# fpusan/moira

Measured on AMD Instinct MI355X. Metric: reads/sec filtered (300 bp synthetic), higher is better.
Workload: dtype f64; 1 GPU; BASELINE configs[1]: 10000000 synthetic single-end 300 bp reads, poisson_binomial filter, alpha 0.005, uncert 0.01, resident in HBM (uint8 10000000 x 320, seed 2); reads_per_gpu=10000000, read_length=300, row_stride=320, parallelism=host-side split, 1 rank(s), no data-path collective, world_size=1, mode=bit-exact (no FMA)

## Files before the change

### include/moira_pb.h

```cpp
#ifndef MOIRA_PB_H
#define MOIRA_PB_H

#include <stdint.h>

#ifdef __cplusplus
extern "C" {
#endif
#if defined(__GNUC__) || defined(__clang__)
#pragma GCC visibility push(default)
#endif

#define MPB_OK            0
#define MPB_E_INVALID    -1
#define MPB_E_NODEVICE   -2
#define MPB_E_HIP        -3
#define MPB_E_NOMEM      -4
#define MPB_E_RANGE      -5

#define MPB_AMBIG_TREAT_AS_ERRORS 0
#define MPB_AMBIG_IGNORE          1
#define MPB_AMBIG_DISALLOW        2

#define MPB_FLAG_ROUND      1u
#define MPB_FLAG_FAST_FMA   2u
// ... 167 lines not shown
int mpb_broker_attach(const char *name, int32_t wait_ms, mpb_broker_client **client_out);
int mpb_broker_call(mpb_broker_client *client, const char *contig, const int32_t *contig_quals, int32_t len,
                    double alpha, double *ee, int32_t *ns);
int mpb_broker_detach(mpb_broker_client *client);
int mpb_broker_shutdown(const char *name);
int mpb_broker_stats(const char *name, int64_t *served, int64_t *batches, int64_t *solo, int32_t *pid, int32_t *attached);

int mpb_numa_cpulist_for_pci(const char *sysfs_root, const char *pci_bus_id, int32_t *node_out, char *cpulist_out, int32_t cpulist_len);

int mpb_poisson_lambda_device(mpb_ctx *ctx, const uint8_t *d_q, int64_t n, int64_t row_stride,
                              const int32_t *d_len, int32_t fixed_len,
                              double *d_lambda, int32_t *d_ns);
int mpb_poisson_finish_host(const double *lambda, const int32_t *ns, const int32_t *len,
                            int32_t fixed_len, int64_t n, const mpb_filter_params *params,
                            double *ee, uint8_t *pass);
int mpb_filter_poisson_host(mpb_ctx *ctx, const uint8_t *q, int64_t n, int64_t row_stride,
                            const int32_t *len, int32_t fixed_len, const mpb_filter_params *params,
                            double *ee, int32_t *ns, uint8_t *pass, mpb_filter_counts *counts);

int mpb_poisson_finish_device(mpb_ctx *ctx, const double *d_lambda, const int32_t *d_ns,
                              const int32_t *d_len, int32_t fixed_len, int64_t n,
                              const mpb_filter_params *params,
                              double *d_ee, uint8_t *d_pass, mpb_filter_counts *counts);
int mpb_filter_poisson_device(mpb_ctx *ctx, const uint8_t *d_q, int64_t n, int64_t row_stride,
                              const int32_t *d_len, int32_t fixed_len,
                              const mpb_filter_params *params,
                              double *d_ee, int32_t *d_ns, uint8_t *d_pass, double *d_lambda,
                              mpb_filter_counts *counts);

int mpb_calculate_errors_poisson(mpb_ctx *ctx, const char *sequence,
                                 const int32_t *quals, int32_t len,
                                 double alpha, double *ee, int32_t *ns);

int mpb_synth_fill_device(mpb_ctx *ctx, uint8_t *d_q, int64_t n, int64_t row_stride,
                          int32_t fixed_len, int32_t min_len, int32_t max_len,
                          int32_t *d_len, uint64_t seed, int64_t first_read);
int mpb_synth_fill_device_profile(mpb_ctx *ctx, uint8_t *d_q, int64_t n, int64_t row_stride,
                                  int32_t fixed_len, int32_t min_len, int32_t max_len,
                                  int32_t *d_len, uint64_t seed, int64_t first_read, int32_t profile);

int mpb_timing_enable(mpb_ctx *ctx, int on);
int mpb_timing_reset(mpb_ctx *ctx);
int mpb_kernel_time(mpb_ctx *ctx, int kernel_id, double *total_ms, int64_t *launches);
int mpb_last_class_histogram(mpb_ctx *ctx, int32_t *caps, int64_t *counts, int32_t max_classes);
int mpb_last_read_budgets(mpb_ctx *ctx, int32_t *caps_out, int64_t n);
int mpb_last_algorithmic_cells(mpb_ctx *ctx, int64_t *cells);

typedef struct mpb_path_info {
    int32_t narrow_rows;
    int32_t sampled;
    int64_t n_fallback;
    int32_t sample_hist[16];
    int32_t narrow_split;
    int32_t reserved_;
} mpb_path_info;
int mpb_last_path(mpb_ctx *ctx, mpb_path_info *out);

#if defined(__GNUC__) || defined(__clang__)
#pragma GCC visibility pop
#endif
#ifdef __cplusplus
}
#endif
#endif
```

### moira_amd/_lib.py

```python
import ctypes as C
import os

_HERE = os.path.dirname(os.path.abspath(__file__))
LIB_PATH = os.path.join(_HERE, "libmoira_pb.so")

MAX_LEN = 65535
OK, E_INVALID, E_NODEVICE, E_HIP, E_NOMEM, E_RANGE = 0, -1, -2, -3, -4, -5
AMBIG = {"treat_as_errors": 0, "ignore": 1, "disallow": 2}
FLAG_ROUND, FLAG_FAST_FMA, FLAG_TEST_UNDERPREDICT, FLAG_DECISION_ONLY, FLAG_BATCHED_ONLY, FLAG_COUNT_CELLS = 1, 2, 4, 8, 16, 32
FLAG_NO_NARROW = 64
FLAG_ODDS = 128
FLAG_ODDS_NARROW = 1 << 20
FLAG_POISSON_DEVICE_TAIL = 1 << 21


def FLAG_NARROW_ROWS(r):
    return (int(r) & 15) << 8


K_PREPASS, K_SCAN, K_SCATTER, K_DP, K_OVERFLOW, K_LAMBDA, K_WIDE, K_NARROW, K_FALLBACK, K_SAMPLE = 0, 1, 2, 3, 4, 5, 6, 7, 8, 9
K_POISSON_TAIL = 10
K_PACK_TEXT = 11
KERNEL_NAMES = {K_PREPASS: "prepass", K_SCAN: "scan", K_SCATTER: "scatter", K_DP: "dp", K_OVERFLOW: "overflow", K_LAMBDA: "lambda",
                K_WIDE: "wide", K_NARROW: "narrow", K_FALLBACK: "fallback", K_SAMPLE: "sample", K_POISSON_TAIL: "poisson_tail",
                K_PACK_TEXT: "pack_text"}


class MoiraPBError(RuntimeError):
    pass


class NoDeviceError(MoiraPBError):
    pass


class FilterParams(C.Structure):
    _fields_ = [("alpha", C.c_double), ("uncert", C.c_double), ("maxerrors", C.c_double),
                ("ambig_mode", C.c_int32), ("flags", C.c_uint32)]


class PathInfo(C.Structure):
    _fields_ = [("narrow_rows", C.c_int32), ("sampled", C.c_int32), ("n_fallback", C.c_int64),
                ("sample_hist", C.c_int32 * 16), ("narrow_split", C.c_int32), ("reserved_", C.c_int32)]


class FilterCounts(C.Structure):
    _fields_ = [("n_reads", C.c_int64), ("n_pass", C.c_int64), ("n_fail", C.c_int64),
                ("n_overflow", C.c_int64)]


class TextRow(C.Structure):
    _fields_ = [("seq_off", C.c_int64), ("qual_off", C.c_int64), ("len", C.c_int32), ("pad", C.c_int32)]


class PairRow(C.Structure):
    _fields_ = [("fseq_off", C.c_int64), ("fqual_off", C.c_int64), ("fhdr_off", C.c_int64), ("rseq_off", C.c_int64),
                ("rqual_off", C.c_int64), ("l1", C.c_int32), ("l2", C.c_int32), ("hdr_len", C.c_int32), ("pad", C.c_int32)]


class ContigParams(C.Structure):
    _fields_ = [(k, C.c_int32) for k in ("match", "mismatch", "gap", "insert", "deltaq", "consensus", "qscore_cap", "trim_overlap")]


CONTIG_MAX_LEN = 384

_VP, _I32P, _U8P, _DP = C.c_void_p, C.POINTER(C.c_int32), C.POINTER(C.c_uint8), C.POINTER(C.c_double)
PROTOTYPES = {
    "mpb_version": (C.c_char_p, []),
    "mpb_last_error": (C.c_char_p, []),
    "mpb_device_count": (C.c_int, []),
    "mpb_create": (C.c_int, [C.c_int, C.POINTER(_VP)]),
    "mpb_destroy": (C.c_int, [_VP]),
    "mpb_host_lut": (C.c_int, [_VP, _VP]),
    "mpb_device_lut": (C.c_int, [_VP, _VP, _VP]),
    "mpb_stream": (C.c_int, [_VP, C.POINTER(_VP)]),
    "mpb_synchronize": (C.c_int, [_VP]),
    "mpb_malloc": (C.c_int, [_VP, C.c_int64, C.POINTER(_VP)]),
    "mpb_free": (C.c_int, [_VP, _VP]),
    "mpb_memcpy_h2d": (C.c_int, [_VP, _VP, _VP, C.c_int64]),
    "mpb_memcpy_d2h": (C.c_int, [_VP, _VP, _VP, C.c_int64]),
    "mpb_memset": (C.c_int, [_VP, _VP, C.c_int, C.c_int64]),
    "mpb_host_alloc": (C.c_int, [_VP, C.c_int64, C.POINTER(_VP)]),
    "mpb_host_free": (C.c_int, [_VP, _VP]),
    "mpb_pack_read": (C.c_int, [C.c_char_p, _VP, C.c_int32, _VP, C.c_int32]),
    "mpb_pack_read_ascii": (C.c_int, [C.c_char_p, C.c_char_p, C.c_int32, C.c_int32, _VP, C.c_int32]),
    "mpb_pack_batch_ascii": (C.c_int, [C.c_char_p, C.c_char_p, _VP, C.c_int64, C.c_int32, C.c_int32, C.c_int64, _VP, _VP]),
    "mpb_decode_ascii_device": (C.c_int, [_VP, _VP, _VP, C.c_int64, C.c_int64, _VP, C.c_int32, C.c_int32, _VP, _VP]),
    "mpb_text_rows": (C.c_int, [_VP, C.c_int64, _VP, C.c_int64, C.c_int64, C.c_int32, C.c_int64, _VP, C.POINTER(C.c_int64),
                                C.POINTER(C.c_int64)]),
    "mpb_pack_text_device": (C.c_int, [_VP, _VP, C.c_int64, _VP, C.c_int64, C.c_int32, C.c_int32, C.c_int64, _VP, _VP, _VP, _VP]),
    "mpb_filter_text_host": (C.c_int, [_VP, _VP, C.c_int64, _VP, C.c_int64, _VP, C.c_int64, C.c_int32, C.c_int32, C.c_int32,
                                       C.POINTER(FilterParams), C.c_int32, _VP, _VP, _VP, _VP, _VP, C.POINTER(FilterCounts),
                                       C.POINTER(C.c_int64)]),
    "mpb_pair_rows": (C.c_int, [_VP, _VP, C.c_int64, C.c_int64, C.c_int64, C.c_int64, _VP, C.POINTER(C.c_int64)]),
    "mpb_contig_posterior_tables": (C.c_int, [_VP, _VP]),
    "mpb_contigs_text_host": (C.c_int, [_VP, _VP, C.c_int64, _VP, _VP, C.c_int64, _VP, C.c_int64, C.c_int32, C.POINTER(ContigParams),
# ... 95 lines not shown
```

### moira_amd/build.py

```python
import fcntl
import hashlib
import os
import subprocess
import sys

HERE = os.path.dirname(os.path.abspath(__file__))
ROOT = os.path.dirname(HERE)
CSRC = os.path.join(HERE, "csrc")
LIB = os.path.join(HERE, "libmoira_pb.so")
HOST_SOURCES = [os.path.join(CSRC, name) for name in ("mpb_hostonly.cpp", "mpb_context.cpp", "mpb_resident.cpp", "mpb_hostfed.cpp",
                                                      "mpb_perread.cpp", "mpb_poisson.cpp", "mpb_text.cpp", "mpb_contig.cpp",
                                                      "mpb_broker.cpp")]
CONTIG_KERNELS = os.path.join(CSRC, "mpb_contig_kernels.hip")
SOURCES = [os.path.join(CSRC, "mpb_kernels.hip"), CONTIG_KERNELS] + HOST_SOURCES
DEPS = SOURCES + [os.path.join(CSRC, "mpb_internal.h"), os.path.join(CSRC, "mpb_host_internal.h"),
                  os.path.join(CSRC, "mpb_shared.h"), os.path.join(CSRC, "mpb_hostonly.h"), os.path.join(CSRC, "mpb_ctx.h"),
                  os.path.join(CSRC, "mpb_dp_tiles.inc"),
                  os.path.join(CSRC, "mpb_narrow_ring.inc"), os.path.join(CSRC, "mpb_narrow_rs.inc"),
                  os.path.join(CSRC, "mpb_narrow_rg.inc"),
                  os.path.join(CSRC, "mpb_contig_lane.inc"), os.path.join(CSRC, "mpb_contig_args.h"),
                  os.path.join(CSRC, "contig_posterior.h"),
                  os.path.join(CSRC, "libmoira_pb.map"),
                  os.path.join(ROOT, "include", "moira_pb.h"),
                  os.path.join(ROOT, "include", "mpb_synth.h")]
HIPCC = os.environ.get("HIPCC", "/opt/rocm/bin/hipcc")
FLAGS = ["-O3", "--offload-arch=gfx950", "-fPIC", "-shared", "-std=c++17",
         "-ffp-contract=off", "-fno-fast-math", "-pthread", "-Wall", "-Wno-unused-function",
         "-Werror=pass-failed",
         "-fvisibility=hidden",
         "-Wl,--version-script=" + os.path.join(CSRC, "libmoira_pb.map"),
         "-x", "hip"]


CONTIG_LIB = os.path.join(HERE, "libmoira_contig.so")
CONTIG_SRC = os.path.join(CSRC, "contig.cpp")
CXX = os.environ.get("CXX", "g++")


CONTIG_DEPS = [CONTIG_SRC, os.path.join(CSRC, "contig_posterior.h"), os.path.join(ROOT, "include", "moira_contig.h"),
               os.path.join(ROOT, "include", "moira_io.h")]


def _digest(paths, flags):
    h = hashlib.sha256(" ".join(flags).encode())
    for p in paths:
        with open(p, "rb") as f:
            h.update(f.read())
    return h.hexdigest()


def _is_stale(lib, deps, flags):
    stamp = lib + ".stamp"
    if not os.path.exists(lib) or not os.path.exists(stamp):
        return True
    try:
        return open(stamp).read().strip() != _digest(deps, flags)
    except OSError:
        return True


def _locked_build(lib, deps, flags, cmd, force, verbose):
    with open(lib + ".lock", "w") as lk:
        fcntl.flock(lk, fcntl.LOCK_EX)
        try:
            if force or _is_stale(lib, deps, flags):
                if verbose:
                    print(" ".join(cmd))
                tmp = lib + ".tmp.%d" % os.getpid()
                subprocess.check_call(cmd[:-1] + [tmp])
                os.replace(tmp, lib)
                with open(lib + ".stamp", "w") as f:
                    f.write(_digest(deps, flags))
                if verbose:
# ... 71 lines not shown
```

### moira_amd/csrc/mpb_internal.h

```cpp
#ifndef MPB_INTERNAL_H
#define MPB_INTERNAL_H

#include <hip/hip_runtime.h>
#include "mpb_shared.h"

#define MPB_TILE_MAX_ROWS 1024
#define MPB_WIDE_WAVES 16
#define MPB_MAX_ROWS (MPB_TILE_MAX_ROWS * MPB_WIDE_WAVES)
#define MPB_MAX_STRIDE 65536
#define MPB_SMALL_MAX_STRIDE 16384

struct MpbClass { int cap, G, R; };

#define MPB_NCLS 32
#define MPB_CLASSES(X)                                                                       \
    X(0, 2, 1) X(1, 3, 1) X(2, 4, 1) X(3, 5, 1) X(4, 6, 1) X(5, 7, 1) X(6, 8, 1) X(7, 9, 1)  \
    X(8, 10, 1) X(9, 12, 1) X(10, 14, 1) X(11, 16, 1)                                        \
    X(12, 10, 2) X(13, 12, 2) X(14, 14, 2) X(15, 16, 2)                                      \
    X(16, 10, 4) X(17, 12, 4) X(18, 14, 4) X(19, 16, 4)                                      \
    X(20, 9, 8) X(21, 10, 8) X(22, 11, 8) X(23, 12, 8) X(24, 14, 8) X(25, 16, 8)             \
    X(26, 10, 16) X(27, 12, 16) X(28, 16, 16)                                                \
    X(29, 12, 32) X(30, 16, 32) X(31, 16, 64)

#define MPB_THIN_CLASSES(X)                                                                  \
// ... 22 lines not shown
};

#define MPB_DP_CHUNK 8

struct MpbDevParams {
    double thr;
    double uncert;
    double maxerrors;
    float  z;
    float  zq;
    float  clow;
    int32_t ambig_mode;
    uint32_t flags;
    int32_t fixed_len;
    int32_t max_len;
    int32_t len_shift;
};

struct MpbWorkspace {
    uint8_t  *cls;
    int32_t  *perm;
    uint16_t *perm_ns;
    int32_t  *blockhist;
    MpbTables *tables;
    MpbTables *tables2;
    int32_t  *ovf_list;
    int32_t  *ovf_count;
    int32_t  *bad_len;
    long long *ovf_total;
    int32_t  *wide_list;
    int32_t  *wide_rows;
    int32_t  *wide_count;
    unsigned long long *pass_count;
    unsigned long long *alg_cells;
    const double2 *lut;
    int32_t  *nar_count;
    int32_t  *nar_seg;
    int32_t  *nar_list;
    int32_t  *nar_wave_count;
    int32_t  *nar_sample;
    int2     *rg_ord;
    int32_t  *rg_gpre;
    unsigned long long *rg_wsum, *rg_wpre;
    int32_t  *rg_gstart;
    int32_t  *pt_count;
};

#define MPB_NAR_MAX_WAVES 8192
#define MPB_NAR_AUTO_MIN_READS (1 << 18)

#define MPB_LUT_BYTES   (256 * 16)
#define MPB_LAMBDA_MAX_STRIDE (1 << 24)

void mpb_launch_prepass(const uint8_t *q, int64_t n, int64_t stride, const int32_t *len,
                        const MpbDevParams &prm, const MpbWorkspace &ws, int32_t *ns_out,
                        double *ee_out, uint8_t *pass_out, hipStream_t s, const int32_t *list = nullptr);
void mpb_launch_decode_classify(const uint8_t *seq, const uint8_t *qual, int32_t offset, uint8_t *out, int32_t *err,
                                int64_t n, int64_t stride, const int32_t *len, const MpbDevParams &prm,
                                const MpbWorkspace &ws, int32_t *ns_out, double *ee_out, uint8_t *pass_out, hipStream_t s);
void mpb_launch_encode(const uint8_t *q, int64_t n, int64_t stride, int32_t offset, uint8_t *seq, uint8_t *qual, hipStream_t s);
struct MpbSmallHost {
    uint8_t *stage;
    int32_t *ns_dev;
    uint32_t *done;
    uint32_t token;
};
void mpb_launch_small(const uint8_t *q, int64_t n, int64_t stride, const int32_t *len, const MpbDevParams &prm,
                      const MpbWorkspace &ws, int32_t *ns, double *ee, uint8_t *pass, hipStream_t s,
                      const MpbSmallHost *host = nullptr);
#define MPB_SERVE_STRIDE 2048
struct alignas(64) MpbServePrm { MpbDevParams p; };
struct MpbServeBox {
    const uint8_t *q;
    int64_t stride;
    const MpbServePrm *prm;
    const unsigned long long *door;
    uint32_t *done;
    double *ee; int32_t *ns; uint8_t *pass;
    int64_t q_step, prm_step, door_step, done_step, ee_step, ns_step, pass_step;
    const uint32_t *stop;
    uint32_t *exited;
    uint8_t *stage;
    int32_t *ns_dev; uint8_t *cls; int32_t *ident;
    uint32_t *gone;
    int32_t n_ent;
};
void mpb_launch_serve(const MpbServeBox &box, const double2 *lut, uint32_t generation, uint32_t lifetime_ms, hipStream_t s);
void mpb_launch_scan(int64_t n, const int32_t *len, const MpbWorkspace &ws, hipStream_t s);
void mpb_launch_scatter(int64_t n, const int32_t *len, const int32_t *ns, const MpbDevParams &prm, const MpbWorkspace &ws,
                        hipStream_t s, const int32_t *list = nullptr);
void mpb_launch_dp(const uint8_t *q, int64_t n, int64_t stride, const int32_t *len,
                   const MpbDevParams &prm, const MpbWorkspace &ws, const int32_t *ns,
                   double *ee, uint8_t *pass, hipStream_t s, const double2 *lut_odds = nullptr);
void mpb_launch_overflow(const uint8_t *q, int64_t n, int64_t stride, const int32_t *len,
                         const MpbDevParams &prm, const MpbWorkspace &ws, const int32_t *ns,
                         double *ee, uint8_t *pass, hipStream_t s);
void mpb_launch_wide(const uint8_t *q, int64_t stride, const int32_t *len, const MpbDevParams &prm,
                     const MpbWorkspace &ws, const int32_t *ns, double *ee, uint8_t *pass, hipStream_t s);
void mpb_launch_lambda(const uint8_t *q, int64_t n, int64_t stride, const int32_t *len, int32_t fixed_len,
                       const double2 *lut_ap, double *lambda, int32_t *ns, int32_t *bad, hipStream_t s);
#define MPB_PT_LAMBDA_MAX 64.0
#define MPB_PT_WINDOW 0x1p-17
struct MpbPoissonRec { double lambda; int32_t idx, ns, len, pad_; };
struct MpbPoissonFix { double ee; int32_t idx, pass; };
void mpb_launch_poisson_tail(const double *lambda, const int32_t *ns, const int32_t *len, int64_t n, const MpbDevParams &prm,
                             double *ee, uint8_t *pass, int32_t *handed, MpbPoissonRec *rec, int32_t rec_cap,
                             unsigned long long *n_pass, hipStream_t s);
// ... 24 lines not shown
```

### moira_amd/csrc/mpb_kernels.hip

```cpp

#include "mpb_internal.h"
#include <cstdlib>
#include <cstdio>
#include "../../include/mpb_synth.h"

#pragma clang fp contract(off)

__shared__ double2 mpb_s_lut[256];
__shared__ unsigned long long mpb_s_cells;

namespace {

__constant__ MpbClass c_classes[MPB_NCLS] = MPB_CLASS_TABLE;

struct ClassOfRows {
    uint8_t t[MPB_TILE_MAX_ROWS + 1];
    constexpr ClassOfRows() : t{}
    {
        constexpr MpbClass cl[MPB_NCLS] = MPB_CLASS_TABLE;
        for (int rows = 0; rows < MPB_TILE_MAX_ROWS + 1; rows++) {
            int c = 0;
            for (int k = 0; k < MPB_NCLS - 1; k++) c += (rows > cl[k].cap) ? 1 : 0;
            t[rows] = (uint8_t)c;
        }
// ... 263 lines not shown
                    y.x = fill_dword(y.x, nv); y.y = fill_dword(y.y, nv - 4);
                    y.z = fill_dword(y.z, nv - 8); y.w = fill_dword(y.w, nv - 12);
                }
                pre_chunk(s_tab, y, a01, s3);
            }
        }
        const float n255 = floorf(a01.y * (1.0f / MPB_MARK_LOWER));
        if (n255 > 0.0f) {
            a01 = (f32x2){0.f, 0.f};
            s3 = 0.f;
#pragma unroll 1
            for (int c0 = pb; c0 < pend; c0 += 4) {
                const int nv = li - (c0 + cl) * 16;
                if (nv <= 0) break;
#pragma unroll 1
                for (int d = 0; d < 4; d++)
                    pre_dword_again(s_tab, fill_dword(*reinterpret_cast<const uint32_t *>(src + c0 * 16 + d * 4), nv - 4 * d), a01, s3);
            }
        }
        const float rem = a01.y;
        const float nzero = floorf(rem * (1.0f / MPB_MARK_UPPER));
        const float pvar = rem - MPB_MARK_UPPER * nzero;
        mu += a01.x;
        var += pvar;
        k3 += pvar - 2.0f * s3;
        ambi += (uint32_t)nzero + ((uint32_t)n255 << 16);
        };
        if (LONG) { for (int pb = 0; pb < ncol; pb += 12 * MPB_PRE_NB) panel(pb, min(ncol, pb + 12 * MPB_PRE_NB)); }
        else panel(0, ncol);
#pragma unroll
        for (int off = 16; off <= 32; off <<= 1) {
            mu += __shfl_xor(mu, off);
            var += __shfl_xor(var, off);
            k3 += __shfl_xor(k3, off);
            ambi += __shfl_xor(ambi, off);
        }
        const float amb = __uint_as_float(ambi);
        if (cl == 0) s_row[w][rb + r16] = make_float4(mu, var, k3, amb);
    }
    wave_lds_fence();
    {
        const int64_t k = wave_row0 + lane;
        if (k < n) {
            const int64_t i = LISTED ? (int64_t)list[k] : k;
            const float4 e = s_row[w][lane];
            const int li = len ? clamp_len(len[i], prm.max_len) : prm.fixed_len;
            class_read(i, e.x, e.y, e.z, __float_as_uint(e.w), li, RAGGED && li != len[i], RAGGED, prm, o, s_hist, nb);
        }
    }
    wave_lds_fence();
    }
    __syncthreads();
    for (int k = tid; k < MPB_NCLS * nb; k += 256) blockhist[(int64_t)k * gridDim.x + blockIdx.x] = s_hist[k];
}

#define MPB_LIN_K 5
#define MPB_LIN_CHUNKS (256 * MPB_LIN_K)

template <bool RAGGED, bool DECODE>
__global__ __launch_bounds__(256) void k_classify_linear(const uint8_t *__restrict__ q, int64_t n, int64_t stride,
                                                         const int32_t *__restrict__ len_arg, MpbDevParams prm, PreOut o,
                                                         int32_t *__restrict__ blockhist, PreDecode dec, uint32_t cpr_magic)
{
    __shared__ float2 s_tab[256];
    __shared__ float4 s_part[MPB_LIN_CHUNKS];
    __shared__ int s_len[MPB_PRE_READS];
    __shared__ int s_hist[RAGGED ? MPB_SKEYS : MPB_NCLS];
    const int32_t *__restrict__ len = RAGGED ? len_arg : nullptr;
    constexpr int nb = RAGGED ? MPB_LEN_BINS : 1;
    const int tid = threadIdx.x;
    {
        const bool amb = tid == 0 || tid == 255;
        float p = __builtin_amdgcn_exp2f(-0.33219281f * (float)tid);
        p = amb ? 0.0f : p;
        s_tab[tid] = make_float2(p, tid == 0 ? MPB_MARK_UPPER : tid == 255 ? MPB_MARK_LOWER : p * (1.0f - p));
    }
    for (int k = tid; k < MPB_NCLS * nb; k += 256) s_hist[k] = 0;
    const int cpr = (int)(stride >> 4);
    const int tile_rows = max(1, min(MPB_PRE_READS, MPB_LIN_CHUNKS / cpr));
    const int64_t first = (int64_t)blockIdx.x * MPB_PRE_READS;
    const int64_t last = min(n, first + MPB_PRE_READS);
    int lpr = 1;
    while (lpr < 64 && lpr * 2 * tile_rows <= 256) lpr *= 2;
    int badq = 0;
    for (int64_t row0 = first; row0 < last; row0 += tile_rows) {
        const int nr = (int)min((int64_t)tile_rows, last - row0);
        const int nchunks = nr * cpr;
        __syncthreads();
        for (int t = tid; t < nr; t += 256) s_len[t] = len ? clamp_len(len[row0 + t], prm.max_len) : prm.fixed_len;
        __syncthreads();
        const int64_t base = row0 * stride;
        uint4 xs[MPB_LIN_K], ys[MPB_LIN_K];
        int nvs[MPB_LIN_K];
#pragma unroll
        for (int k = 0; k < MPB_LIN_K; k++) {
            const int c = tid + k * 256;
            xs[k] = ys[k] = make_uint4(0, 0, 0, 0);
            nvs[k] = -1;
            if (c < nchunks) {
                const int r = cpr_magic ? (int)__umulhi((uint32_t)c, cpr_magic) : c;
                const int col = c - r * cpr;
                const int nv = s_len[r] - col * 16;
                nvs[k] = max(nv, 0);
                if (nv > 0) {
                    if (DECODE) {
                        xs[k] = *reinterpret_cast<const uint4 *>(dec.seq + base + (int64_t)c * 16);
// ... 1629 lines not shown
            y.z = fill_dword(y.z, nv - 8); y.w = fill_dword(y.w, nv - 12);
            pre_chunk(s_tab, y, a01, s3);
            const uint32_t ww[4] = {y.x, y.y, y.z, y.w};
#pragma unroll
            for (int d = 0; d < 4; d++)
#pragma unroll
                for (int t = 0; t < 4; t++) {
                    const float4 e = s_pow[(ww[d] >> (8 * t)) & 0xffu];
                    lp0 += e.x; t1 += e.y; t2 += e.z; t3 += e.w;
                }
        }
        const float n255 = floorf(a01.y * (1.0f / MPB_MARK_LOWER));
        const float rem = a01.y - MPB_MARK_LOWER * n255;
        const float nzero = floorf(rem * (1.0f / MPB_MARK_UPPER));
        const float pvar = rem - MPB_MARK_UPPER * nzero;
        mu += a01.x; var += pvar; k3 += pvar - 2.0f * s3;
        ambi += (int)nzero + (int)n255;
        lower += (int)n255;
    }
#pragma unroll
    for (int off = 1; off <= 32; off <<= 1) {
        mu += __shfl_xor(mu, off); var += __shfl_xor(var, off);
        k3 += __shfl_xor(k3, off); ambi += __shfl_xor(ambi, off); lower += __shfl_xor(lower, off);
        lp0 += __shfl_xor(lp0, off); t1 += __shfl_xor(t1, off);
        t2 += __shfl_xor(t2, off); t3 += __shfl_xor(t3, off);
    }
    if (lane == 0) {
        const float vv = fmaxf(var, 1e-12f);
        const float x = mu + prm.z * sqrtf(vv) + (k3 / vv) * prm.zq;
        int rows = (int)floorf(fminf(x, 1e9f) + 0.5f) + 1;
        rows = max(rows, 5);
        const float thr = (float)prm.thr;
        const float p0 = __expf(lp0);
        const float e1 = t1, e2 = 0.5f * (t1 * t1 - t2), e3 = (t1 * t1 * t1 - 3.0f * t1 * t2 + 2.0f * t3) * (1.0f / 6.0f);
        float cdf = p0;
        if (cdf > thr) rows = 1;
        else if ((cdf += p0 * e1) > thr) rows = 2;
        else if ((cdf += p0 * e2) > thr) rows = 3;
        else if ((cdf += p0 * e3) > thr) rows = 4;
        rows = max(min(rows, li - ambi + 1), 1);
        atomicAdd(hist + ((lower > 0 || bad_len) ? 0 : min(rows, MPB_NAR_BUCKETS - 1)),
                  len ? max(1, (li + 15) >> 4) : 1);
        if (len && lower == 0 && !bad_len) {
            if (rows >= 3) atomicMin(hist + MPB_NAR_BUCKETS, (li + 15) >> 4);
            if (rows >= 4) atomicMin(hist + MPB_NAR_BUCKETS + 1, (li + 15) >> 4);
        }
    }
}

}

static inline int pre_blocks(int64_t n) { return (int)((n + MPB_PRE_READS - 1) / MPB_PRE_READS); }

void mpb_launch_prepass(const uint8_t *q, int64_t n, int64_t stride, const int32_t *len,
                        const MpbDevParams &prm, const MpbWorkspace &ws, int32_t *ns_out,
                        double *ee_out, uint8_t *pass_out, hipStream_t s, const int32_t *list)
{
#define MPB_PRE_LAUNCH(RG, LG, LS)                                                                                      \
    hipLaunchKernelGGL((k_prepass<RG, LG, LS>), dim3(pre_blocks(n)), dim3(256), 0, s, q, n, stride, len, prm, o, ws.blockhist, list)
    const PreOut o = {ws.cls, ns_out, ee_out, pass_out, ws.bad_len, ws.wide_list, ws.wide_rows, ws.wide_count};
    const bool long_rows = prm.max_len > 16 * 12 * MPB_PRE_NB;
    if (list) {
        if (len) { if (long_rows) MPB_PRE_LAUNCH(true, true, true); else MPB_PRE_LAUNCH(true, false, true); }
        else     { if (long_rows) MPB_PRE_LAUNCH(false, true, true); else MPB_PRE_LAUNCH(false, false, true); }
    } else {
        if (len) { if (long_rows) MPB_PRE_LAUNCH(true, true, false); else MPB_PRE_LAUNCH(true, false, false); }
        else     { if (long_rows) MPB_PRE_LAUNCH(false, true, false); else MPB_PRE_LAUNCH(false, false, false); }
    }
#undef MPB_PRE_LAUNCH
}

void mpb_launch_decode_classify(const uint8_t *seq, const uint8_t *qual, int32_t offset, uint8_t *out, int32_t *err,
                                int64_t n, int64_t stride, const int32_t *len, const MpbDevParams &prm,
                                const MpbWorkspace &ws, int32_t *ns_out, double *ee_out, uint8_t *pass_out, hipStream_t s)
{
    const PreOut o = {ws.cls, ns_out, ee_out, pass_out, ws.bad_len, ws.wide_list, ws.wide_rows, ws.wide_count};
    const PreDecode dec = {seq, qual, out, offset, err};
    const uint8_t *q = out;
    const uint32_t cpr = (uint32_t)(stride >> 4);
    const uint32_t magic = cpr == 1 ? 0u : (uint32_t)(((1ull << 32) + cpr - 1) / cpr);
    if (len) hipLaunchKernelGGL((k_classify_linear<true, true>), dim3(pre_blocks(n)), dim3(256), 0, s, q, n, stride, len, prm, o, ws.blockhist, dec, magic);
    else     hipLaunchKernelGGL((k_classify_linear<false, true>), dim3(pre_blocks(n)), dim3(256), 0, s, q, n, stride, len, prm, o, ws.blockhist, dec, magic);
}

void mpb_launch_encode(const uint8_t *q, int64_t n, int64_t stride, int32_t offset, uint8_t *seq, uint8_t *qual, hipStream_t s)
{
    const int64_t chunks = n * (stride / 16);
    hipLaunchKernelGGL(k_encode_ascii, dim3((unsigned)((chunks + 255) / 256)), dim3(256), 0, s, q, n, stride, offset, seq, qual);
}

void mpb_launch_scan(int64_t n, const int32_t *len, const MpbWorkspace &ws, hipStream_t s)
{
    const int nb = len ? MPB_LEN_BINS : 1;
    hipLaunchKernelGGL(k_scan, dim3(MPB_NCLS * nb), dim3(256), 0, s, ws.blockhist, pre_blocks(n), ws.tables);
    hipLaunchKernelGGL(k_tables, dim3(1), dim3(512), 0, s, ws.tables, nb, ws.ovf_count, ws.pass_count);
}

void mpb_launch_scatter(int64_t n, const int32_t *len, const int32_t *ns, const MpbDevParams &prm, const MpbWorkspace &ws,
                        hipStream_t s, const int32_t *list)
{
    if (len)
        hipLaunchKernelGGL((k_scatter<true>), dim3(pre_blocks(n)), dim3(256), 0, s, ws.cls, n, len, prm.max_len, prm.len_shift,
                           ws.blockhist, ws.tables, ns, ws.perm, ws.perm_ns, list);
    else
        hipLaunchKernelGGL((k_scatter<false>), dim3(pre_blocks(n)), dim3(256), 0, s, ws.cls, n, len, prm.max_len, prm.len_shift,
                           ws.blockhist, ws.tables, ns, ws.perm, ws.perm_ns, list);
}

#define MPB_DP_GRID (1 << 20)


static DpArgs make_args(const uint8_t *q, int64_t stride, const int32_t *len, const MpbDevParams &prm,
                        const MpbWorkspace &ws, const int32_t *ns, double *ee, uint8_t *pass, int final_pass)
{
    DpArgs A;
    A.q = q; A.stride = stride; A.len = len; A.ns = ns; A.cls = ws.cls; A.ee = ee; A.pass = pass;
    A.ovf_list = ws.ovf_list; A.ovf_count = ws.ovf_count; A.alg_cells = ws.alg_cells; A.prm = prm; A.final_pass = final_pass;
    A.perm = ws.perm; A.perm_ns = final_pass == 0 ? ws.perm_ns : nullptr;
    return A;
}

void mpb_launch_dp(const uint8_t *q, int64_t n, int64_t stride, const int32_t *len,
// ... 275 lines not shown
```

### moira_amd/csrc/mpb_resident.cpp

```cpp

#include "mpb_ctx.h"

#include <cmath>
#include <cstring>


MpbDevParams make_dev_params(const mpb_filter_params *p, int32_t fixed_len, int32_t max_len)
{
    MpbDevParams d;
    d.thr = 1 - p->alpha;
    d.uncert = p->uncert;
    d.maxerrors = p->maxerrors;
    const double z = inv_norm_cdf(1 - p->alpha);
    d.z = (float)z;
    d.zq = (float)((z * z - 1) / 6);
    if (!(z == z) || std::isinf(z)) { d.z = 1e30f; d.zq = 0.0f; }
    d.clow = (float)(sqrt(2 * log(1 / (1 - p->alpha))) * 1.0001);
    d.ambig_mode = p->ambig_mode;
    d.flags = p->flags;
    d.fixed_len = fixed_len;
    d.max_len = max_len;
    d.len_shift = MPB_LEN_SHIFT;
    while (((max_len - 1) >> d.len_shift) >= MPB_LEN_BINS) d.len_shift++;
    return d;
// ... 34 lines not shown
    unsigned long long *np = &c->pin->n_pass;
    int32_t *novf = &c->pin->n_overflow, *bad = &c->pin->bad_len;
    *novf = *bad = 0;
    if (!sorted) HIPCHK(hipMemsetAsync(c->ws.pass_count, 0, sizeof(unsigned long long), s));
    mpb_launch_count(d_pass, n, c->ws, s);
    HIPCHK(hipMemcpyAsync(np, c->ws.pass_count, sizeof(*np), hipMemcpyDeviceToHost, s));
    if (sorted) HIPCHK(hipMemcpyAsync(novf, c->ws.ovf_count, sizeof(*novf), hipMemcpyDeviceToHost, s));
    if (d_len) HIPCHK(hipMemcpyAsync(bad, c->ws.bad_len, sizeof(*bad), hipMemcpyDeviceToHost, s));
    HIPCHK(hipStreamSynchronize(s));
    if (*bad) {
        HIPCHK(hipMemsetAsync(c->ws.bad_len, 0, sizeof(int32_t), s));
        return fail(MPB_E_INVALID, "%d read length(s) in d_len outside 0..%d (row_stride %lld; reads longer than %d bases "
                    "are not supported); those reads were given ee = NaN, pass = 0", *bad, max_len, (long long)row_stride, MPB_MAX_LEN);
    }
    counts->n_pass = (int64_t)*np;
    counts->n_fail = n - (int64_t)*np;
    counts->n_overflow = *novf;
    return MPB_OK;
}

static int filter_device_tail(mpb_ctx *c, const uint8_t *d_q, int64_t n, int64_t row_stride, const int32_t *d_len,
                              const MpbDevParams &prm, double *d_ee, int32_t *d_ns, uint8_t *d_pass, mpb_filter_counts *counts,
                              const int32_t *d_list = nullptr)
{
    hipStream_t s = c->stream;
    const int32_t max_len = prm.max_len;
    { Span t(c, MPB_K_SCAN);     mpb_launch_scan(n, d_len, c->ws, s); }
    { Span t(c, MPB_K_SCATTER);  mpb_launch_scatter(n, d_len, d_ns, prm, c->ws, s, d_list); }
    const double2 *lut_odds = (prm.flags & MPB_FLAG_ODDS) && c->ws.lut == c->d_lut ? c->d_lut_odds : nullptr;
    { Span t(c, MPB_K_DP);       mpb_launch_dp(d_q, n, row_stride, d_len, prm, c->ws, d_ns, d_ee, d_pass, s, lut_odds); }
    if (max_len + 1 > MPB_TILE_MAX_ROWS) { Span t(c, MPB_K_WIDE); mpb_launch_wide(d_q, row_stride, d_len, prm, c->ws, d_ns, d_ee, d_pass, s); }
    { Span t(c, MPB_K_OVERFLOW); mpb_launch_overflow(d_q, n, row_stride, d_len, prm, c->ws, d_ns, d_ee, d_pass, s); }
    HIPCHK(hipGetLastError());
    return counts ? fetch_counts(c, n, row_stride, d_len, max_len, d_pass, true, counts) : MPB_OK;
}

static bool narrow_eligible(const mpb_ctx *c, int64_t n, int64_t row_stride, const int32_t *d_len, int32_t fixed_len, const mpb_filter_params *p)
{
    uint32_t forbidden = MPB_FLAG_FAST_FMA | MPB_FLAG_ODDS | MPB_FLAG_TEST_UNDERPREDICT | MPB_FLAG_DECISION_ONLY | MPB_FLAG_COUNT_CELLS | MPB_FLAG_NO_NARROW;
    if (p->flags & MPB_FLAG_ODDS_NARROW) forbidden &= ~MPB_FLAG_ODDS;
    if (!(c->narrow_ok && n >= 1 && !(p->flags & forbidden) && c->ws.lut == c->d_lut)) return false;
    return d_len ? row_stride <= MPB_RG_MAX_STRIDE : fixed_len >= 1;
}

static int filter_device_general(mpb_ctx *c, const uint8_t *d_q, int64_t n, int64_t row_stride, const int32_t *d_len,
                                 int32_t fixed_len, int32_t max_len, const mpb_filter_params *params,
                                 double *d_ee, int32_t *d_ns, uint8_t *d_pass, mpb_filter_counts *counts,
                                 const int32_t *d_list = nullptr, int64_t n_matrix = 0)
{
    int rc;
    if ((rc = prepare_batch(c, d_list && n_matrix > n ? n_matrix : n, max_len))) return rc;
    const MpbDevParams prm = make_dev_params(params, fixed_len, max_len);
    if (params->flags & MPB_FLAG_COUNT_CELLS) HIPCHK(hipMemsetAsync(c->ws.alg_cells, 0, sizeof(unsigned long long), c->stream));
    { Span t(c, MPB_K_PREPASS);  mpb_launch_prepass(d_q, n, row_stride, d_len, prm, c->ws, d_ns, d_ee, d_pass, c->stream, d_list); }
    return filter_device_tail(c, d_q, n, row_stride, d_len, prm, d_ee, d_ns, d_pass, counts, d_list);
}

static int narrow_choose(mpb_ctx *c, const uint8_t *d_q, int64_t n, int64_t row_stride, const int32_t *d_len, int32_t fixed_len,
                         const mpb_filter_params *params, const MpbDevParams &prm, int *rows0, int *split)
{
    *rows0 = 0;
    *split = 0;
    c->last_path.sampled = 0;
    const int forced = (int)((params->flags >> 8) & 15u);
    if (forced) {
        *rows0 = forced < MPB_NAR_MIN_ROWS ? MPB_NAR_MIN_ROWS : forced > MPB_NAR_MAX_ROWS ? MPB_NAR_MAX_ROWS : forced;
        *split = d_len && !(params->flags & MPB_FLAG_ODDS_NARROW) ? (int)((params->flags >> 12) & 255u) : 0;
        return MPB_OK;
    }
    if (n < MPB_NAR_AUTO_MIN_READS) return MPB_OK;
    auto &ch = c->nar_choice;
    if (d_len) fixed_len = -1;
    const bool same = ch.valid && ch.n == n && ch.stride == row_stride && ch.fixed_len == fixed_len &&
                      memcmp(&ch.alpha, &params->alpha, sizeof(double)) == 0 && ch.flags == params->flags;
    if (same && ch.calls < 64) { ch.calls++; *rows0 = ch.rows0; *split = ch.split; return MPB_OK; }
    int n_sample = (int)(n / 1024 < 256 ? 256 : n / 1024 > 4096 ? 4096 : n / 1024);
    { Span t(c, MPB_K_SAMPLE); mpb_launch_sample(d_q, n, row_stride, fixed_len, d_len, prm, c->ws, n_sample, c->stream); }
    HIPCHK(hipMemcpyAsync(c->pin->sample, c->ws.nar_sample, sizeof(c->pin->sample), hipMemcpyDeviceToHost, c->stream));
    HIPCHK(hipStreamSynchronize(c->stream));
    c->last_path.sampled = 1;
    const int32_t *sample = c->pin->sample;
    int weight = 0;
    for (int k = 0; k < MPB_NAR_BUCKETS; k++) { c->last_path.sample_hist[k] = sample[k]; weight += sample[k]; }
    const bool odds = (params->flags & MPB_FLAG_ODDS_NARROW) != 0;
    *rows0 = narrow_rows_from_sample(sample, weight, odds);
    if (d_len && *rows0 >= 3 && !odds) {
        const int need = sample[MPB_NAR_BUCKETS + (*rows0 - 3)];
        if (need > 0 && need < (1 << 20)) {
            const int cut = need - 1 - need / 16;
            if (cut >= 4) *split = cut > 255 ? 255 : cut;
        }
    }
    ch.split = *split;
    {
        double back = sample[0];
        for (int r = *rows0 + 1; r < MPB_NAR_BUCKETS; r++) back += sample[r];
        ch.expect_back = weight > 0 ? back / weight : 0.0;
    }
    ch.valid = true; ch.n = n; ch.stride = row_stride; ch.fixed_len = fixed_len; ch.alpha = params->alpha; ch.flags = params->flags;
    ch.rows0 = *rows0; ch.calls = 0;
    return MPB_OK;
}

static int filter_device_narrow(mpb_ctx *c, int rows0, int split, const uint8_t *d_q, int64_t n, int64_t row_stride, const int32_t *d_len,
                                int32_t fixed_len, const mpb_filter_params *params, const MpbDevParams &prm,
                                double *d_ee, int32_t *d_ns, uint8_t *d_pass, mpb_filter_counts *counts)
{
// ... 216 lines not shown
```

### moira_amd/engine.py

```python
import ctypes as C
import math

import numpy as np

from . import _lib as L


def _round_up(x, m):
    return (x + m - 1) // m * m


class DeviceBuffer:

    def __init__(self, engine, nbytes):
        self.engine, self.nbytes = engine, int(nbytes)
        p = C.c_void_p()
        L.check(engine.lib.mpb_malloc(engine.ctx, self.nbytes, C.byref(p)))
        self.ptr = p.value

    def upload(self, arr):
        arr = np.ascontiguousarray(arr)
        assert arr.nbytes <= self.nbytes
        L.check(self.engine.lib.mpb_memcpy_h2d(self.engine.ctx, self.ptr, arr.ctypes.data, arr.nbytes))
        return self
# ... 383 lines not shown
    def poisson_finish_device(self, d_lambda, d_ns, n, d_len=None, fixed_len=0, d_ee=None, d_pass=None, params=None,
                              want_counts=True):
        params = params or self.params()
        ptr = lambda b: (b.ptr if isinstance(b, DeviceBuffer) else b)
        counts = L.FilterCounts()
        L.check(self.lib.mpb_poisson_finish_device(self.ctx, ptr(d_lambda), ptr(d_ns), ptr(d_len) if d_len is not None else None,
                                                   int(fixed_len), n, C.byref(params), ptr(d_ee), ptr(d_pass),
                                                   C.byref(counts) if want_counts else None))
        return counts if want_counts else None

    def filter_poisson_device(self, d_q, n, stride, d_len=None, fixed_len=0, d_ee=None, d_ns=None, d_pass=None, d_lambda=None,
                              params=None, want_counts=True):
        params = params or self.params()
        ptr = lambda b: (b.ptr if isinstance(b, DeviceBuffer) else b)
        counts = L.FilterCounts()
        L.check(self.lib.mpb_filter_poisson_device(self.ctx, ptr(d_q), n, stride, ptr(d_len) if d_len is not None else None,
                                                   int(fixed_len), C.byref(params), ptr(d_ee), ptr(d_ns), ptr(d_pass),
                                                   ptr(d_lambda) if d_lambda is not None else None,
                                                   C.byref(counts) if want_counts else None))
        return counts if want_counts else None

    def calculate_errors_PB(self, contig, contig_quals, alpha):
        from .broker import marshal_read
        seq, qi, addr, alpha = marshal_read(contig, contig_quals, alpha)
        ee, ns = C.c_double(), C.c_int32()
        L.check(self.lib.mpb_calculate_errors_PB(self.ctx, seq, addr, len(qi), alpha,
                                                 C.byref(ee), C.byref(ns)))
        return ee.value, ns.value

    def calculate_errors_poisson(self, sequence, quals, alpha):
        sequence = str(sequence)
        qi = np.array([int(v) for v in quals], np.int64).astype(np.int32) if len(quals) else np.empty(0, np.int32)
        alpha = float(alpha)
        if len(sequence) != len(qi):
            raise ValueError("sequence and quals must have the same length")
        if alpha <= 0 or alpha >= 1:
            raise ValueError("Alpha must be between 0 (not included) and 1.")
        ee, ns = C.c_double(), C.c_int32()
        L.check(self.lib.mpb_calculate_errors_poisson(self.ctx, sequence.encode(), qi.ctypes.data, len(qi), alpha,
                                                      C.byref(ee), C.byref(ns)))
        if ee.value != ee.value:
            raise OverflowError("Lambda ** expected_errors or its factorial leaves the float range (moira.py:1671)")
        return ee.value, ns.value

    def synth_fill(self, d_q, n, stride, fixed_len=0, min_len=0, max_len=0, d_len=None, seed=1, first_read=0, profile=0):
        ptr = lambda b: (b.ptr if isinstance(b, DeviceBuffer) else b)
        L.check(self.lib.mpb_synth_fill_device_profile(self.ctx, ptr(d_q), n, stride, fixed_len, min_len, max_len,
                                                       ptr(d_len) if d_len is not None else None, seed, first_read, profile))

    def last_path(self):
        info = L.PathInfo()
        L.check(self.lib.mpb_last_path(self.ctx, C.byref(info)))
        return {"narrow_rows": info.narrow_rows, "sampled": bool(info.sampled), "n_fallback": info.n_fallback,
                "sample_hist": list(info.sample_hist), "narrow_split": info.narrow_split}

    def timing(self, on=True):
        L.check(self.lib.mpb_timing_enable(self.ctx, 1 if on else 0))

    def timing_reset(self):
        L.check(self.lib.mpb_timing_reset(self.ctx))

    def kernel_times(self):
        out = {}
        for kid, name in L.KERNEL_NAMES.items():
            ms, cnt = C.c_double(), C.c_int64()
            L.check(self.lib.mpb_kernel_time(self.ctx, kid, C.byref(ms), C.byref(cnt)))
            out[name] = (ms.value, cnt.value)
        return out

    def device_lut(self):
        a, b = np.empty(256), np.empty(256)
        L.check(self.lib.mpb_device_lut(self.ctx, a.ctypes.data, b.ctypes.data))
        return a, b

    def algorithmic_cells(self):
        v = C.c_int64()
        L.check(self.lib.mpb_last_algorithmic_cells(self.ctx, C.byref(v)))
        return v.value

    def read_budgets(self, n):
        out = np.empty(n, np.int32)
        L.check(self.lib.mpb_last_read_budgets(self.ctx, out.ctypes.data, n))
        return out

    def class_histogram(self):
        caps = np.zeros(64, np.int32)
        cnts = np.zeros(64, np.int64)
        k = self.lib.mpb_last_class_histogram(self.ctx, caps.ctypes.data, cnts.ctypes.data, 64)
        if k < 0:
            L.check(k)
        return {int(caps[i]): int(cnts[i]) for i in range(k)}


def host_lut():
    a, b = np.empty(256), np.empty(256)
    L.check(L.load().mpb_host_lut(a.ctypes.data, b.ctypes.data))
    return a, b


_default_engine = None


def default_engine():
    global _default_engine
    if _default_engine is None:
        import os
        _default_engine = Engine(int(os.environ.get("LOCAL_RANK", "0")))
# ... 2 lines not shown
```

Before: 2.585 billion reads/s.

## Add cache-line-aligned prepass kernel for fixed-length strided resident reads

```diff
diff --git a/include/moira_pb.h b/include/moira_pb.h
--- a/include/moira_pb.h
+++ b/include/moira_pb.h
@@ -243,7 +243,7 @@
     int64_t n_fallback;
     int32_t sample_hist[16];
     int32_t narrow_split;
-    int32_t reserved_;
+    int32_t prepass_lines;
 } mpb_path_info;
 int mpb_last_path(mpb_ctx *ctx, mpb_path_info *out);
 
diff --git a/moira_amd/_lib.py b/moira_amd/_lib.py
--- a/moira_amd/_lib.py
+++ b/moira_amd/_lib.py
@@ -41,7 +41,7 @@
 
 class PathInfo(C.Structure):
     _fields_ = [("narrow_rows", C.c_int32), ("sampled", C.c_int32), ("n_fallback", C.c_int64),
-                ("sample_hist", C.c_int32 * 16), ("narrow_split", C.c_int32), ("reserved_", C.c_int32)]
+                ("sample_hist", C.c_int32 * 16), ("narrow_split", C.c_int32), ("prepass_lines", C.c_int32)]
 
 
 class FilterCounts(C.Structure):
diff --git a/moira_amd/build.py b/moira_amd/build.py
--- a/moira_amd/build.py
+++ b/moira_amd/build.py
@@ -19,6 +19,7 @@
                   os.path.join(CSRC, "mpb_narrow_ring.inc"), os.path.join(CSRC, "mpb_narrow_rs.inc"),
                   os.path.join(CSRC, "mpb_narrow_rg.inc"),
                   os.path.join(CSRC, "mpb_contig_lane.inc"), os.path.join(CSRC, "mpb_contig_args.h"),
+                  os.path.join(CSRC, "mpb_prepass_lines.inc"),
                   os.path.join(CSRC, "contig_posterior.h"),
                   os.path.join(CSRC, "libmoira_pb.map"),
                   os.path.join(ROOT, "include", "moira_pb.h"),
diff --git a/moira_amd/csrc/mpb_internal.h b/moira_amd/csrc/mpb_internal.h
--- a/moira_amd/csrc/mpb_internal.h
+++ b/moira_amd/csrc/mpb_internal.h
@@ -98,7 +98,7 @@
 #define MPB_LUT_BYTES   (256 * 16)
 #define MPB_LAMBDA_MAX_STRIDE (1 << 24)
 
-void mpb_launch_prepass(const uint8_t *q, int64_t n, int64_t stride, const int32_t *len,
+bool mpb_launch_prepass(const uint8_t *q, int64_t n, int64_t stride, const int32_t *len,
                         const MpbDevParams &prm, const MpbWorkspace &ws, int32_t *ns_out,
                         double *ee_out, uint8_t *pass_out, hipStream_t s, const int32_t *list = nullptr);
 void mpb_launch_decode_classify(const uint8_t *seq, const uint8_t *qual, int32_t offset, uint8_t *out, int32_t *err,
diff --git a/moira_amd/csrc/mpb_kernels.hip b/moira_amd/csrc/mpb_kernels.hip
--- a/moira_amd/csrc/mpb_kernels.hip
+++ b/moira_amd/csrc/mpb_kernels.hip
@@ -339,6 +339,193 @@
     }
     __syncthreads();
     for (int k = tid; k < MPB_NCLS * nb; k += 256) blockhist[(int64_t)k * gridDim.x + blockIdx.x] = s_hist[k];
+}
+
+#define PL_FN __host__ __device__ __forceinline__
+#include "mpb_prepass_lines.inc"
+#define MPB_PL_NB 5
+#define MPB_PL_EDGES 3
+
+template <int CTRL>
+__device__ __forceinline__ float pl_dpp(float x)
+{
+    return __int_as_float(__builtin_amdgcn_update_dpp(0, __float_as_int(x), CTRL, 0xf, 0xf, true));
+}
+struct PlSums { float mu, var, k3; uint32_t ambi; };
+__device__ __forceinline__ void pl_fold_quad(PlSums &v)
+{
+    v.mu += pl_dpp<0x4E>(v.mu); v.var += pl_dpp<0x4E>(v.var); v.k3 += pl_dpp<0x4E>(v.k3);
+    v.ambi += (uint32_t)__builtin_amdgcn_update_dpp(0, (int)v.ambi, 0x4E, 0xf, 0xf, true);
+    v.mu += pl_dpp<0xB1>(v.mu); v.var += pl_dpp<0xB1>(v.var); v.k3 += pl_dpp<0xB1>(v.k3);
+    v.ambi += (uint32_t)__builtin_amdgcn_update_dpp(0, (int)v.ambi, 0xB1, 0xf, 0xf, true);
+}
+__device__ __forceinline__ PlSums pl_mirror(const PlSums &v)
+{
+    PlSums r;
+    r.mu = pl_dpp<0x141>(v.mu); r.var = pl_dpp<0x141>(v.var); r.k3 = pl_dpp<0x141>(v.k3);
+    r.ambi = (uint32_t)__builtin_amdgcn_update_dpp(0, (int)v.ambi, 0x141, 0xf, 0xf, true);
+    return r;
+}
+
+template <int K>
+__global__ __launch_bounds__(256) void k_prepass_lines(const uint8_t *__restrict__ q, int64_t n, int64_t stride,
+                                                       MpbDevParams prm, PreOut o, int32_t *__restrict__ blockhist)
+{
+    __shared__ float2 s_tab[256];
+    __shared__ float4 s_row[4][64];
+    __shared__ int s_hist[MPB_NCLS];
+    const int tid = threadIdx.x, lane = tid & 63;
+    const int w = __builtin_amdgcn_readfirstlane(tid >> 6);
+    {
+        const bool amb = tid == 0 || tid == 255;
+        float p = __builtin_amdgcn_exp2f(-0.33219281f * (float)tid);
+        p = amb ? 0.0f : p;
+        s_tab[tid] = make_float2(p, tid == 0 ? MPB_MARK_UPPER : tid == 255 ? MPB_MARK_LOWER : p * (1.0f - p));
+    }
+    for (int k = tid; k < MPB_NCLS; k += 256) s_hist[k] = 0;
+    __syncthreads();
+
+    const PlShape S = pl_shape((int)stride, prm.fixed_len);
+    const int li = S.li;
+    const int c8 = lane & 7;
+    const bool lo = c8 < 4;
+    uint32_t load_bits = 0;
+    int edge_line[MPB_PL_EDGES] = {-1, -1, -1};
+    uint32_t keep[MPB_PL_EDGES][4];
+#pragma unroll
+    for (int e = 0; e < MPB_PL_EDGES; e++)
+#pragma unroll
+        for (int d = 0; d < 4; d++) keep[e][d] = 0xffffffffu;
+    {
+        int e = 0;
+        for (int p = 0; p < S.np; p++) {
+            const int kind = pl_line_kind(S, p);
+            if (kind != PL_SKIP) load_bits |= 1u << p;
+            if (kind != PL_EDGE) continue;
+#pragma unroll
+            for (int f = 0; f < MPB_PL_EDGES; f++)
+                if (f == e) edge_line[f] = p;
+            const int nv = pl_nvalid(S, p, lane);
+#pragma unroll
+            for (int d = 0; d < 4; d++) {
+                const uint32_t m = mask_dword(0xffffffffu, nv - 4 * d);
+#pragma unroll
+                for (int f = 0; f < MPB_PL_EDGES; f++)
+                    if (f == e) keep[f][d] = m;
+            }
+            e++;
+        }
+    }
+    const int lane_off = (lane >> 3) * S.kb + c8 * 16;
+
+    for (int round = 0; round < MPB_PRE_ROUNDS; round++) {
+    const int64_t wave_row0 = (int64_t)blockIdx.x * MPB_PRE_READS + round * 256 + w * 64;
+    if (wave_row0 >= n) break;
+    const int rows_here = (int)min((int64_t)PL_WAVE_ROWS, n - wave_row0);
+    const uint64_t base = (uint64_t)(uintptr_t)q + (uint64_t)wave_row0 * (uint64_t)stride;
+    const uint32_t b_lo = (uint32_t)__builtin_amdgcn_readfirstlane((int)(uint32_t)base);
+    const uint32_t b_hi = (uint32_t)__builtin_amdgcn_readfirstlane((int)(uint32_t)(base >> 32));
+    const uint32_t b_n = (uint32_t)__builtin_amdgcn_readfirstlane(rows_here * S.stride);
+    const __amdgpu_buffer_rsrc_t rsrc = __builtin_amdgcn_make_buffer_rsrc(
+        (void *)(uintptr_t)(((uint64_t)b_hi << 32) | b_lo), 0, (int)b_n, 0x00020000);
+    const int groups = pl_groups_here(S, rows_here);
+
+    for (int g = 0; g < groups; g++) {
+        const int gbase = g * 8 * S.kb;
+        const int goff = lane_off + gbase;
+        f32x2 acc = {0.f, 0.f}, acc_a = {0.f, 0.f};
+        float s3 = 0.f, s3_a = 0.f;
+        for (int pb = 0; pb < S.np; pb += MPB_PL_NB) {
+            u32x4 xs[MPB_PL_NB];
+#pragma unroll
+            for (int b = 0; b < MPB_PL_NB; b++) {
+                const int far = ((load_bits >> (pb + b)) & 1u) ? 0 : (1 << 30);
+                xs[b] = __builtin_amdgcn_raw_buffer_load_b128(rsrc, goff + (pb + b) * 128 + far, 0, 0);
+            }
+            __builtin_amdgcn_sched_barrier(0);
+#pragma unroll
+            for (int b = 0; b < MPB_PL_NB; b++) {
+                const int p = pb + b;
+                if (p >= S.np) break;
+                const bool loaded = (load_bits >> p) & 1u;
+                uint4 y = make_uint4(xs[b].x, xs[b].y, xs[b].z, xs[b].w);
+#pragma unroll
+                for (int e = 0; e < MPB_PL_EDGES; e++)
+                    if (p == edge_line[e]) {
+                        y.x = (y.x & keep[e][0]) | (0xFEFEFEFEu & ~keep[e][0]); y.y = (y.y & keep[e][1]) | (0xFEFEFEFEu & ~keep[e][1]);
+                        y.z = (y.z & keep[e][2]) | (0xFEFEFEFEu & ~keep[e][2]); y.w = (y.w & keep[e][3]) | (0xFEFEFEFEu & ~keep[e][3]);
+                    }
+                if (K == 2 && p == S.h) {
+                    f32x2 t01 = {0.f, 0.f};
+                    float t3 = 0.f;
+                    if (loaded) pre_chunk(s_tab, y, t01, t3);
+                    acc_a = acc + (lo ? t01 : (f32x2){0.f, 0.f});
+                    s3_a = s3 + (lo ? t3 : 0.f);
+                    acc = lo ? (f32x2){0.f, 0.f} : t01;
+                    s3 = lo ? 0.f : t3;
+                } else if (loaded) {
+                    pre_chunk(s_tab, y, acc, s3);
+                }
+            }
+        }
+        auto peel = [&](f32x2 a01, float t3, const int second, const bool both) {
+            const float n255 = floorf(a01.y * (1.0f / MPB_MARK_LOWER));
+            if (n255 > 0.0f) {
+                a01 = (f32x2){0.f, 0.f};
+                t3 = 0.f;
+#pragma unroll 1
+                for (int side = 0; side < (both ? 2 : 1); side++) {
+                    const int ln = side ? (lane ^ 7) : lane;
+                    const int off = (ln >> 3) * S.kb + (ln & 7) * 16 + gbase;
+#pragma unroll 1
+                    for (int p = 0; p < S.np; p++) {
+                        const int nv = pl_nvalid(S, p, ln);
+                        if (pl_second(S, p, ln) != second || nv <= 0) continue;
+#pragma unroll 1
+                        for (int d = 0; d < 4; d++) {
+                            const uint32_t x = __builtin_amdgcn_raw_buffer_load_b32(rsrc, off + p * 128 + d * 4, 0, 0);
+                            pre_dword_again(s_tab, fill_dword(x, nv - 4 * d), a01, t3);
+                        }
+                    }
+                }
+            }
+            const float rem = a01.y;
+            const float nzero = floorf(rem * (1.0f / MPB_MARK_UPPER));
+            const float pvar = rem - MPB_MARK_UPPER * nzero;
+            PlSums r;
+            r.mu = a01.x; r.var = pvar; r.k3 = pvar - 2.0f * t3;
+            r.ambi = (uint32_t)nzero + ((uint32_t)n255 << 16);
+            return r;
+        };
+        if (K == 2) {
+            f32x2 mine01 = lo ? acc_a : acc, send01 = lo ? acc : acc_a;
+            float mine3 = lo ? s3_a : s3;
+            const float send3 = lo ? s3 : s3_a;
+            mine01.x += pl_dpp<0x141>(send01.x); mine01.y += pl_dpp<0x141>(send01.y); mine3 += pl_dpp<0x141>(send3);
+            PlSums mine = peel(mine01, mine3, lo ? 0 : 1, true);
+            pl_fold_quad(mine);
+            if ((c8 & 3) == 0)
+                s_row[w][(g * 8 + (lane >> 3)) * 2 + (c8 >> 2)] = make_float4(mine.mu, mine.var, mine.k3, __uint_as_float(mine.ambi));
+        } else {
+            PlSums mine = peel(acc, s3, 0, false);
+            const PlSums got = pl_mirror(mine);
+            mine.mu += got.mu; mine.var += got.var; mine.k3 += got.k3; mine.ambi += got.ambi;
+            pl_fold_quad(mine);
+            if (c8 == 0) s_row[w][g * 8 + (lane >> 3)] = make_float4(mine.mu, mine.var, mine.k3, __uint_as_float(mine.ambi));
+        }
+    }
+    wave_lds_fence();
+    {
+        const int64_t i = wave_row0 + lane;
+        if (i < n) {
+            const float4 e = s_row[w][lane];
+            class_read(i, e.x, e.y, e.z, __float_as_uint(e.w), li, false, false, prm, o, s_hist, 1);
+        }
+    }
+    wave_lds_fence();
+    }
+    __syncthreads();
+    for (int k = tid; k < MPB_NCLS; k += 256) blockhist[(int64_t)k * gridDim.x + blockIdx.x] = s_hist[k];
 }
 
 #define MPB_LIN_K 5
@@ -2074,7 +2261,7 @@
 
 static inline int pre_blocks(int64_t n) { return (int)((n + MPB_PRE_READS - 1) / MPB_PRE_READS); }
 
-void mpb_launch_prepass(const uint8_t *q, int64_t n, int64_t stride, const int32_t *len,
+bool mpb_launch_prepass(const uint8_t *q, int64_t n, int64_t stride, const int32_t *len,
                         const MpbDevParams &prm, const MpbWorkspace &ws, int32_t *ns_out,
                         double *ee_out, uint8_t *pass_out, hipStream_t s, const int32_t *list)
 {
@@ -2082,6 +2269,11 @@
     hipLaunchKernelGGL((k_prepass<RG, LG, LS>), dim3(pre_blocks(n)), dim3(256), 0, s, q, n, stride, len, prm, o, ws.blockhist, list)
     const PreOut o = {ws.cls, ns_out, ee_out, pass_out, ws.bad_len, ws.wide_list, ws.wide_rows, ws.wide_count};
     const bool long_rows = prm.max_len > 16 * 12 * MPB_PRE_NB;
+    if (!list && !len && pl_applies(stride, prm.fixed_len)) {
+        if (stride & 127) hipLaunchKernelGGL((k_prepass_lines<2>), dim3(pre_blocks(n)), dim3(256), 0, s, q, n, stride, prm, o, ws.blockhist);
+        else              hipLaunchKernelGGL((k_prepass_lines<1>), dim3(pre_blocks(n)), dim3(256), 0, s, q, n, stride, prm, o, ws.blockhist);
+        return true;
+    }
     if (list) {
         if (len) { if (long_rows) MPB_PRE_LAUNCH(true, true, true); else MPB_PRE_LAUNCH(true, false, true); }
         else     { if (long_rows) MPB_PRE_LAUNCH(false, true, true); else MPB_PRE_LAUNCH(false, false, true); }
@@ -2090,6 +2282,7 @@
         else     { if (long_rows) MPB_PRE_LAUNCH(false, true, false); else MPB_PRE_LAUNCH(false, false, false); }
     }
 #undef MPB_PRE_LAUNCH
+    return false;
 }
 
 void mpb_launch_decode_classify(const uint8_t *seq, const uint8_t *qual, int32_t offset, uint8_t *out, int32_t *err,
diff --git a/moira_amd/csrc/mpb_prepass_lines.inc b/moira_amd/csrc/mpb_prepass_lines.inc
--- /dev/null
+++ b/moira_amd/csrc/mpb_prepass_lines.inc
@@ -0,0 +1,63 @@
+
+#define PL_MAX_STRIDE 960
+#define PL_WAVE_ROWS 64
+#define PL_SKIP 0
+#define PL_FULL 1
+#define PL_EDGE 2
+
+struct PlShape { int stride, li, k, kb, np, h, groups; };
+
+PL_FN bool pl_applies(long long stride, int li)
+{
+    return stride >= 64 && stride <= PL_MAX_STRIDE && stride % 64 == 0 && li >= 0 && li <= stride;
+}
+
+PL_FN PlShape pl_shape(int stride, int li)
+{
+    PlShape s;
+    s.stride = stride; s.li = li;
+    s.k = (stride & 127) ? 2 : 1;
+    s.kb = s.k * stride;
+    s.np = s.kb >> 7;
+    s.h = s.k == 2 ? (stride >> 7) : -1;
+    s.groups = 8 / s.k;
+    return s;
+}
+
+PL_FN int pl_offset(const PlShape &s, int g, int p, int lane)
+{
+    return (g * 8 + (lane >> 3)) * s.kb + p * 128 + (lane & 7) * 16;
+}
+
+PL_FN int pl_second(const PlShape &s, int p, int lane)
+{
+    return (s.k == 2 && p * 128 + (lane & 7) * 16 >= s.stride) ? 1 : 0;
+}
+
+PL_FN int pl_read(const PlShape &s, int g, int p, int lane)
+{
+    return (g * 8 + (lane >> 3)) * s.k + pl_second(s, p, lane);
+}
+
+PL_FN int pl_nvalid(const PlShape &s, int p, int lane)
+{
+    return s.li - (p * 128 + (lane & 7) * 16 - pl_second(s, p, lane) * s.stride);
+}
+
+PL_FN int pl_half_bases(const PlShape &s, int p, int hf)
+{
+    const int off = p * 128 + hf * 64;
+    const int nv = s.li - (off >= s.stride ? off - s.stride : off);
+    return nv < 0 ? 0 : nv > 64 ? 64 : nv;
+}
+
+PL_FN int pl_line_kind(const PlShape &s, int p)
+{
+    const int b = pl_half_bases(s, p, 0) + pl_half_bases(s, p, 1);
+    return b == 0 ? PL_SKIP : b == 128 ? PL_FULL : PL_EDGE;
+}
+
+PL_FN int pl_groups_here(const PlShape &s, int rows_here)
+{
+    return (rows_here + 8 * s.k - 1) / (8 * s.k);
+}
diff --git a/moira_amd/csrc/mpb_resident.cpp b/moira_amd/csrc/mpb_resident.cpp
--- a/moira_amd/csrc/mpb_resident.cpp
+++ b/moira_amd/csrc/mpb_resident.cpp
@@ -110,7 +110,7 @@
     if ((rc = prepare_batch(c, d_list && n_matrix > n ? n_matrix : n, max_len))) return rc;
     const MpbDevParams prm = make_dev_params(params, fixed_len, max_len);
     if (params->flags & MPB_FLAG_COUNT_CELLS) HIPCHK(hipMemsetAsync(c->ws.alg_cells, 0, sizeof(unsigned long long), c->stream));
-    { Span t(c, MPB_K_PREPASS);  mpb_launch_prepass(d_q, n, row_stride, d_len, prm, c->ws, d_ns, d_ee, d_pass, c->stream, d_list); }
+    { Span t(c, MPB_K_PREPASS);  c->last_path.prepass_lines = mpb_launch_prepass(d_q, n, row_stride, d_len, prm, c->ws, d_ns, d_ee, d_pass, c->stream, d_list) ? 1 : 0; }
     return filter_device_tail(c, d_q, n, row_stride, d_len, prm, d_ee, d_ns, d_pass, counts, d_list);
 }
 
diff --git a/moira_amd/engine.py b/moira_amd/engine.py
--- a/moira_amd/engine.py
+++ b/moira_amd/engine.py
@@ -459,7 +459,7 @@
         info = L.PathInfo()
         L.check(self.lib.mpb_last_path(self.ctx, C.byref(info)))
         return {"narrow_rows": info.narrow_rows, "sampled": bool(info.sampled), "n_fallback": info.n_fallback,
-                "sample_hist": list(info.sample_hist), "narrow_split": info.narrow_split}
+                "sample_hist": list(info.sample_hist), "narrow_split": info.narrow_split, "prepass_lines": bool(info.prepass_lines)}
 
     def timing(self, on=True):
         L.check(self.lib.mpb_timing_enable(self.ctx, 1 if on else 0))
```

Measured after the change: 2.576 billion reads/s. Within noise of the previous version (-0.3%).
